# michael-fonder/M4Depth

Hardware: AMD Instinct MI355X
Metric: frames/s (higher is better)
Workload: dtype f32

## Files before the change

include/m4depth_hip.h:

```cpp
#ifndef M4DEPTH_HIP_H_
#define M4DEPTH_HIP_H_

#include <stdint.h>

#ifdef __cplusplus
extern "C" {
#endif

#define M4D_ABI_VERSION 6

int m4d_abi_version(void);
long long m4d_launch_count(void);
const char* m4d_build_info(void);


int m4d_backproject_fwd(const float* input, const float* coords, const int dims[6],
                        float* out, void* stream);

int m4d_backproject_bwd(const float* grad, const float* input, const float* coords,
                        const int dims[6], float* input_grad, float* coords_grad, void* stream);


int m4d_dense_image_warp(const float* image, const float* flow, int B, int H, int W, int C,
                         float* out, int32_t* index_out, void* stream);
// ... 181 lines not shown
                   float* parallax, float* depth, float* other, float* depth_state, void* stream);

int m4d_bias_act(const float* x, const float* bias, long long rows, int C, float slope,
                 float* out, void* stream);

int m4d_bias_act_padded(const float* x, const float* bias, int b, int h, int w, int C, float slope,
                        float* out, int out_h, int out_w, int off_y, int off_x, void* stream);

int m4d_conv3x3_bias_act(const float* x, const float* wp, const float* bias, int b, int h, int w,
                         int Cin, int Cout, int CoutPad, float slope, float* out, void* stream);
long long m4d_conv3x3_workspace_floats(int b, int h, int w, int CoutPad);
int m4d_conv3x3s_bias_act_ws(const float* x, const float* wp, const float* bias, int b, int h, int w,
                             int Cin, int Cout, int CoutPad, int stride, float slope, float* out,
                             float* workspace, long long workspace_floats, void* stream);
int m4d_conv3x3_bias_act_ws(const float* x, const float* wp, const float* bias, int b, int h, int w,
                            int Cin, int Cout, int CoutPad, float slope, float* out, float* workspace,
                            long long workspace_floats, void* stream);
int m4d_conv3x3_lat(const float* x, int s_in, long long x_slab_floats, const float* x_bias, float x_slope,
                    const void* wp, const float* bias, int b, int h, int w, int Cin, int Cout, float slope,
                    int mt, int kw, int s_out, float* out, long long out_slab_floats, void* stream);
int m4d_conv3x3s_lat(const float* x, int s_in, long long x_slab_floats, const float* x_bias, float x_slope,
                     const void* wp, const float* bias, int b, int h, int w, int Cin, int Cout, int stride, float slope,
                     int mt, int kw, int s_out, float* out, long long out_slab_floats, void* stream);
int m4d_partial_finish(const float* x, int s_in, long long x_slab_floats, const float* bias, float slope,
                       long long pixels, int C, float* out, void* stream);

int m4d_conv3x3_small_bias_act(const float* x, const float* wp, const float* bias, int b, int h, int w,
                               int Cin, int Cout, int CoutPad, float slope, float* out, void* stream);
int m4d_conv3x3s_small_bias_act(const float* x, const float* wp, const float* bias, int b, int h, int w,
                                int Cin, int Cout, int CoutPad, int stride, float slope, float* out, void* stream);
int m4d_conv3x3_small6_bias_act(const float* x, const void* wp6, const float* bias, int b, int h, int w,
                                int Cin, int Cout, int CoutPad, float slope, float* out, void* stream);

long long m4d_dinl_workspace_floats(int b, int C);
int m4d_dinl_fwd_padded(const float* x, const float* scale, const float* bias, int b, int h, int w, int C,
                        float slope, float* workspace, float* out, int out_h, int out_w, int off_y,
                        int off_x, void* stream);
int m4d_dinl_fwd(const float* x, const float* scale, const float* bias, int b, int h, int w, int C,
                 float slope, float* workspace, float* out, void* stream);

int m4d_enc_level0_fwd(const float* images, int bsz, long long stride_b, long long stride_t,
                       const float* w1_hwio, const float* bias1, const float* dn_scale, const float* dn_bias,
                       float dn_slope, const float* w2_hwio, const float* bias2, float slope,
                       int b, int h, int w, float* workspace, float* out, void* stream);
int m4d_enc_level0_stats(const float* images, int bsz, long long stride_b, long long stride_t,
                         const float* w1_hwio, const float* bias1, int b, int h, int w, float* workspace,
// ... 36 lines not shown
```

m4depth_amd/_lib.py:

```python
from __future__ import annotations

import ctypes
import os

import torch

_HERE = os.path.dirname(os.path.abspath(__file__))
LIB_FLAVOUR = os.environ.get("M4D_LIB_FLAVOUR", "product")
LIB_PATH = os.path.join(_HERE, "libm4depth_hip_exp.so" if LIB_FLAVOUR == "experiments" else "libm4depth_hip.so")

ABI_VERSION = 6

_c_fp = ctypes.c_void_p
_c_int = ctypes.c_int
_c_f = ctypes.c_float

class NormLevel(ctypes.Structure):
    _fields_ = [("x", ctypes.c_void_p), ("out", ctypes.c_void_p), ("pixels", ctypes.c_longlong), ("C", ctypes.c_int),
                ("nbre_cuts", ctypes.c_int)]


class ResetLevel(ctypes.Structure):
    _fields_ = [("features", ctypes.c_void_p), ("state_features", ctypes.c_void_p), ("depth_state", ctypes.c_void_p),
                ("parallax", ctypes.c_void_p), ("depth", ctypes.c_void_p), ("other", ctypes.c_void_p),
# ... 35 lines not shown
    "m4d_decode_rgb8_resize": [_c_fp, _c_int, _c_int, _c_int, _c_int, _c_int, _c_fp, _c_fp],
    "m4d_decode_depth_resize": [_c_fp, _c_int, _c_int, _c_int, _c_int, _c_int, _c_int, _c_fp, ctypes.POINTER(_c_int),
                                _c_fp, _c_fp],
    "m4d_normalize_cuts": [_c_fp, _c_int, _c_int, _c_int, _c_int, _c_int, _c_fp, _c_fp],
    "m4d_resize_bilinear_v1": [_c_fp, _c_int, _c_int, _c_int, _c_int, _c_int, _c_int, _c_f, _c_fp, _c_fp],
    "m4d_resize_nearest": [_c_fp, _c_int, _c_int, _c_int, _c_int, _c_int, _c_int, _c_fp, _c_fp],
    "m4d_bias_act": [_c_fp, _c_fp, ctypes.c_longlong, _c_int, _c_f, _c_fp, _c_fp],
    "m4d_dinl_fwd": [_c_fp, _c_fp, _c_fp, _c_int, _c_int, _c_int, _c_int, _c_f, _c_fp, _c_fp, _c_fp],
    "m4d_dinl_fwd_padded": [_c_fp, _c_fp, _c_fp, _c_int, _c_int, _c_int, _c_int, _c_f, _c_fp, _c_fp,
                            _c_int, _c_int, _c_int, _c_int, _c_fp],
    "m4d_bias_act_padded": [_c_fp, _c_fp, _c_int, _c_int, _c_int, _c_int, _c_f, _c_fp, _c_int, _c_int, _c_int, _c_int, _c_fp],
    "m4d_conv3x3_bias_act": [_c_fp, _c_fp, _c_fp, _c_int, _c_int, _c_int, _c_int, _c_int, _c_int, _c_f, _c_fp, _c_fp],
    "m4d_conv3x3_bias_act_ws": [_c_fp, _c_fp, _c_fp, _c_int, _c_int, _c_int, _c_int, _c_int, _c_int, _c_f, _c_fp,
                                _c_fp, ctypes.c_longlong, _c_fp],
    "m4d_conv3x3s_bias_act_ws": [_c_fp, _c_fp, _c_fp, _c_int, _c_int, _c_int, _c_int, _c_int, _c_int, _c_int, _c_f,
                                 _c_fp, _c_fp, ctypes.c_longlong, _c_fp],
    "m4d_conv3x3_small_bias_act": [_c_fp, _c_fp, _c_fp, _c_int, _c_int, _c_int, _c_int, _c_int, _c_int, _c_f, _c_fp, _c_fp],
    "m4d_conv3x3s_small_bias_act": [_c_fp, _c_fp, _c_fp, _c_int, _c_int, _c_int, _c_int, _c_int, _c_int, _c_int, _c_f, _c_fp, _c_fp],
    "m4d_conv3x3_small6_bias_act": [_c_fp, _c_fp, _c_fp, _c_int, _c_int, _c_int, _c_int, _c_int, _c_int, _c_f, _c_fp, _c_fp],
    "m4d_conv3x3_lat": [_c_fp, _c_int, ctypes.c_longlong, _c_fp, _c_f, _c_fp, _c_fp, _c_int, _c_int, _c_int, _c_int, _c_int, _c_f,
                        _c_int, _c_int, _c_int, _c_fp, ctypes.c_longlong, _c_fp],
    "m4d_conv3x3s_lat": [_c_fp, _c_int, ctypes.c_longlong, _c_fp, _c_f, _c_fp, _c_fp, _c_int, _c_int, _c_int, _c_int, _c_int, _c_int,
                         _c_f, _c_int, _c_int, _c_int, _c_fp, ctypes.c_longlong, _c_fp],
    "m4d_partial_finish": [_c_fp, _c_int, ctypes.c_longlong, _c_fp, _c_f, ctypes.c_longlong, _c_int, _c_fp, _c_fp],
    "m4d_conv3x3_wino_bias_act": [_c_fp, _c_fp, _c_fp, _c_int, _c_int, _c_int, _c_int, _c_int, _c_int, _c_f, _c_fp, _c_fp],
    "m4d_conv3x3_wino2_bias_act": [_c_fp, _c_fp, _c_fp, _c_int, _c_int, _c_int, _c_int, _c_int, _c_int, _c_f, _c_fp, _c_fp],
    "m4d_conv3x3_wino6_bias_act": [_c_fp, _c_fp, _c_fp, _c_int, _c_int, _c_int, _c_int, _c_int, _c_int, _c_f, _c_fp, _c_fp],
    "m4d_conv3x3_wino6_bias_act_k": [_c_fp, _c_fp, _c_fp, _c_int, _c_int, _c_int, _c_int, _c_int, _c_int, _c_f, _c_fp, _c_int, _c_fp],
    "m4d_conv3x3_wino6_bias_act_ks": [_c_fp, _c_fp, _c_fp, _c_int, _c_int, _c_int, _c_int, _c_int, _c_int, _c_f, _c_fp, _c_int,
                                      _c_int, _c_int, _c_fp],
    "m4d_conv3x3_winof16_bias_act_ks": [_c_fp, _c_fp, _c_fp, _c_int, _c_int, _c_int, _c_int, _c_int, _c_int, _c_f, _c_fp,
                                        _c_int, _c_int, _c_fp],
    "m4d_enc_head_fwd": [_c_fp, _c_int, ctypes.c_longlong, ctypes.c_longlong, _c_fp, _c_fp, _c_int, _c_int, _c_int, _c_int,
                         _c_fp, _c_fp, _c_fp],
    "m4d_enc_level0_stats": [_c_fp, _c_int, ctypes.c_longlong, ctypes.c_longlong, _c_fp, _c_fp, _c_int, _c_int, _c_int, _c_fp, _c_fp, _c_fp,
                             _c_fp],
    "m4d_enc_level0_apply": [_c_fp, _c_int, ctypes.c_longlong, ctypes.c_longlong, _c_fp, _c_fp, _c_fp, _c_fp, _c_fp, _c_fp, _c_f, _c_fp,
                             _c_fp, _c_f, _c_int, _c_int, _c_int, _c_fp, _c_fp],
    "m4d_enc_level0_fwd": [_c_fp, _c_int, ctypes.c_longlong, ctypes.c_longlong, _c_fp, _c_fp, _c_fp, _c_fp, _c_f, _c_fp, _c_fp, _c_f,
                           _c_int, _c_int, _c_int, _c_fp, _c_fp, _c_fp],
    "m4d_conv3x3s2_dinl_bias_act": [_c_fp, _c_fp, _c_fp, _c_fp, _c_fp, _c_f, _c_fp, _c_fp, _c_int, _c_int, _c_int, _c_int, _c_int,
                                    _c_f, _c_fp, _c_fp],
    "m4d_refiner_tail": [_c_fp, _c_fp, _c_fp, _c_fp, _c_fp, _c_fp, _c_int, _c_fp, _c_fp, _c_fp, _c_int, _c_int, _c_int, _c_f,
                         _c_fp, _c_fp, _c_fp, _c_fp, _c_fp],
    "m4d_refiner_tail6": [_c_fp, _c_fp, _c_fp, _c_fp, _c_fp, _c_fp, _c_int, _c_fp, _c_fp, _c_fp, _c_int, _c_int, _c_int, _c_f,
                          _c_fp, _c_fp, _c_fp, _c_fp, _c_fp],
# ... 153 lines not shown
```

m4depth_amd/csrc/m4d_convlat.hip:

```cpp
#include <cstdlib>
#include "m4d_common.h"
#include "../../include/m4depth_hip.h"

namespace {

typedef float lat_f32x16 __attribute__((ext_vector_type(16)));
typedef __bf16 lat_bf16x8 __attribute__((ext_vector_type(8)));

struct LatArgs {
  const float* x; long long x_slab; int s_in;
  const float* x_bias; float x_slope;
  const unsigned char* wp;
  const float* bias; float slope;
  float* out; long long out_slab; int s_out;
  int b, h, w, Cin, Cout, n_chunks, n_groups, tiles_x, tiles_y;
  int cgw_log2, chunks_per_slice;
  int oh, ow, pad_y, pad_x;
};

constexpr int kLatRow = 24;

template <int SIN, int HW, int HP>
__device__ __forceinline__ void lat_stage(const LatArgs& a, float* lds_a, int t, int bi, int gy0, int gx0, int c0, int n_st) {
  constexpr int IB = SIN >= 3 ? 2 : 4;
  const int n_items = n_st * HP * 4;
  for (int base = 0; base < n_items; base += 256 * IB) {
    float4 v[IB][SIN];
    int dst[IB], ch[IB];
    bool ok[IB];
#pragma unroll
    for (int i = 0; i < IB; ++i) {
      const int idx = base + i * 256 + t;
      const int idc = min(idx, n_items - 1);
      const int j = idc / (HP * 4), rem = idc - j * (HP * 4);
      const int hp = rem >> 2, q = rem & 3;
      const int gy = gy0 + hp / HW, gx = gx0 + hp % HW;
      ch[i] = (c0 + j) * 16 + 4 * q;
      ok[i] = idx < n_items && gy >= 0 && gy < a.h && gx >= 0 && gx < a.w && ch[i] < a.Cin;
      dst[i] = idx < n_items ? (j * HP + hp) * kLatRow + 2 * q : -1;
      const long long off = (((long long)bi * a.h + min(max(gy, 0), a.h - 1)) * a.w + min(max(gx, 0), a.w - 1)) * a.Cin
                            + min(ch[i], a.Cin - 4);
#pragma unroll
      for (int s = 0; s < SIN; ++s) v[i][s] = *reinterpret_cast<const float4*>(a.x + s * a.x_slab + off);
// ... 165 lines not shown
    v.x += bb.x; v.y += bb.y; v.z += bb.z; v.w += bb.w;
    v.x = v.x > 0.f ? v.x : v.x * slope; v.y = v.y > 0.f ? v.y : v.y * slope;
    v.z = v.z > 0.f ? v.z : v.z * slope; v.w = v.w > 0.f ? v.w : v.w * slope;
    reinterpret_cast<float4*>(out)[i] = v;
  }
}

template <int MTX, int MTY, int STRIDE, bool MW = false>
int lat_launch(const LatArgs& a, int kw_in, hipStream_t s) {
  constexpr int HP = ((8 * MTX - 1) * STRIDE + 3) * ((4 * MTY - 1) * STRIDE + 3), MT = MTX * MTY;
  const int kw = MW ? 1 : kw_in;
  const int cgw = MW ? 1 : 4 / kw;
  const size_t lds_a = (size_t)2 * kw * HP * kLatRow * 4;
  const size_t lds_r = (size_t)(kw - 1) * cgw * MT * 16 * 64 * 4;
  const size_t lds = lds_a > lds_r ? lds_a : lds_r;
  if (lds > 64 * 1024) M4D_LDS_OPT_IN(&conv3x3_lat_kernel<MTX, MTY, STRIDE, MW>);
  const dim3 grid((unsigned)(a.b * a.tiles_x * a.tiles_y), (unsigned)((a.n_groups + cgw - 1) / cgw), (unsigned)a.s_out);
  m4d_launch(conv3x3_lat_kernel<MTX, MTY, STRIDE, MW>, grid, dim3(256), lds, s, a);
  return 0;
}

}

static int lat_make_args(LatArgs& a, int& kw, const float* x, int s_in, long long x_slab_floats, const float* x_bias, float x_slope,
                         const void* wp, const float* bias, int b, int h, int w, int Cin, int Cout, int stride, float slope,
                         int mt, int s_out, float* out, long long out_slab_floats) {
  M4D_CHECK_ARG(x && wp && bias && out && b > 0 && h > 0 && w > 0 && (stride == 1 || stride == 2));
  M4D_CHECK_ARG(Cin >= 16 && Cin % 4 == 0 && Cout >= 1);
  const int oh = (h + stride - 1) / stride, ow = (w + stride - 1) / stride;
  M4D_CHECK_ARG(s_in >= 1 && s_in <= 4 && (s_in == 1 || x_slab_floats >= (long long)b * h * w * Cin));
  M4D_CHECK_ARG(s_out >= 1 && (s_out == 1 || out_slab_floats >= (long long)b * oh * ow * Cout));
  M4D_CHECK_ARG((mt == 1 || mt == 2 || mt == 4 || mt == 8) && (kw == 1 || kw == 2 || kw == 4));
  if (mt == 8) kw = 1;
  a.x = x; a.x_slab = x_slab_floats; a.s_in = s_in; a.x_bias = x_bias; a.x_slope = x_slope;
  a.wp = reinterpret_cast<const unsigned char*>(wp); a.bias = bias; a.slope = slope;
  a.out = out; a.out_slab = out_slab_floats; a.s_out = s_out;
  a.b = b; a.h = h; a.w = w; a.Cin = Cin; a.Cout = Cout; a.oh = oh; a.ow = ow;
  a.pad_y = ((oh - 1) * stride + 3 - h > 0 ? (oh - 1) * stride + 3 - h : 0) / 2;
  a.pad_x = ((ow - 1) * stride + 3 - w > 0 ? (ow - 1) * stride + 3 - w : 0) / 2;
  a.n_chunks = (Cin + 15) / 16; a.n_groups = (Cout + 31) / 32;
  M4D_CHECK_ARG(s_out <= a.n_chunks);
  a.cgw_log2 = kw == 1 ? 2 : (kw == 2 ? 1 : 0);
  a.chunks_per_slice = (a.n_chunks + s_out - 1) / s_out;
  M4D_CHECK_ARG((long long)(s_out - 1) * a.chunks_per_slice < a.n_chunks);
  const int mtx = mt >= 4 ? 2 : 1, mty = mt >= 2 ? 2 : 1;
  a.tiles_x = (ow + 8 * mtx - 1) / (8 * mtx); a.tiles_y = (oh + 4 * mty - 1) / (4 * mty);
  const size_t lds_a = (size_t)2 * kw * ((8 * mtx - 1) * stride + 3) * ((4 * mty - 1) * stride + 3) * kLatRow * 4;
  M4D_CHECK_ARG(lds_a <= 160 * 1024);
  return 0;
}

static int lat_launch_any(const float* x, int s_in, long long x_slab_floats, const float* x_bias, float x_slope,
                          const void* wp, const float* bias, int b, int h, int w, int Cin, int Cout, int stride, float slope,
                          int mt, int kw, int s_out, float* out, long long out_slab_floats, void* stream) {
  LatArgs a;
  const int rc = lat_make_args(a, kw, x, s_in, x_slab_floats, x_bias, x_slope, wp, bias, b, h, w, Cin, Cout, stride, slope, mt, s_out,
                               out, out_slab_floats);
  if (rc) return rc;
  hipStream_t s = (hipStream_t)stream;
  int rl;
  if (stride == 1) {
    if (mt == 1) rl = lat_launch<1, 1, 1>(a, kw, s);
    else if (mt == 2) rl = lat_launch<1, 2, 1>(a, kw, s);
    else if (mt == 4) rl = lat_launch<2, 2, 1>(a, kw, s);
    else rl = lat_launch<2, 2, 1, true>(a, kw, s);
  } else {
    if (mt == 1) rl = lat_launch<1, 1, 2>(a, kw, s);
    else if (mt == 2) rl = lat_launch<1, 2, 2>(a, kw, s);
    else if (mt == 4) rl = lat_launch<2, 2, 2>(a, kw, s);
    else rl = lat_launch<2, 2, 2, true>(a, kw, s);
  }
  if (rl) return rl;
  return M4D_LAUNCH_RESULT();
}
// ... 26 lines not shown
```

m4depth_amd/network.py:

```python
from __future__ import annotations

import ctypes
from collections import namedtuple

import numpy as np
import torch

from . import network_ops as nops
from ._lib import lib, dptr, stream_ptr, check, as_f32
from .synthetic import ENCODER_CHANNELS, REFINER_CHANNELS, f_input_channels, nbre_cuts_for

M4depthAblationParameters = namedtuple('M4depthAblationParameters',
                                       ('DINL', 'SNCV', 'time_recurr', 'normalize_features',
                                        'subdivide_features', 'level_memory'),
                                       defaults=(True, True, True, True, True, True))

_CV_ACCUM = {"fp32_round": 0, "fp16_seq": 1}

import os as _os

kernel_timer = None
debug_tap = None
winograd_conv = _os.environ.get("M4D_WINOGRAD", "1") == "1"

# ... 45 lines not shown
    n32 = -(-cout // 32)
    t16 = b * (-(-h // 16)) * (-(-w // 16))
    if conv_arith in _SPLIT_ARITHS and cin % 16 == 0 and cin >= 32 and cout >= wino6_min_cout and t16 * (-(-cout // 64)) >= wino6_min_workgroups:
        return 6
    if cin % 4 == 0 and t16 * n32 >= winograd2_min_workgroups:
        return 2
    t8 = b * (-(-h // 8)) * (-(-w // 16))
    if cout % 64 == 0 and t8 * (cout // 64) >= 400:
        return 1
    if cout >= 96 and 400 <= t8 * n32 <= 3000:
        return 1
    return 0


pad_refiner_input = _os.environ.get("M4D_PAD_REFINER_INPUT", "1") == "1"

small_map_conv_pixels = int(_os.environ.get("M4D_CONV_SMALL_PX", "2048"))
small_map_stride2 = _os.environ.get("M4D_CONV_SMALL_S2", "1") == "1"

lat_conv_max_pixels = int(_os.environ.get("M4D_LAT_CONV_PX", "2048"))
lat_conv_narrow_max_pixels = int(_os.environ.get("M4D_LAT_CONV_NARROW_PX", "0"))
lat_conv_s2_max_pixels = int(_os.environ.get("M4D_LAT_CONV_S2_PX", "0"))
lat_conv_mw_max_pixels = int(_os.environ.get("M4D_LAT_CONV_MW_PX", "0"))

fused_cost_volumes = _os.environ.get("M4D_FUSED_COST_VOLUMES", "1") == "1"
small_level_front = _os.environ.get("M4D_SMALL_LEVEL_FRONT", "1") == "1"
fused_level_front = _os.environ.get("M4D_FUSED_LEVEL_FRONT", "1") == "1"

fused_front = _os.environ.get("M4D_FUSED_FRONT", "1") == "1"
fused_front_min_pixels = int(_os.environ.get("M4D_FUSED_FRONT_MIN_PX", "0"))
fused_front_coarse_min_pixels = int(_os.environ.get("M4D_FUSED_FRONT_COARSE_MIN_PX", "6000"))

fused_encoder_head = _os.environ.get("M4D_FUSED_ENCODER_HEAD", "1") == "1"

fused_refiner_tail = _os.environ.get("M4D_FUSED_TAIL", "1") == "1"

level_pipeline_streams = int(_os.environ.get("M4D_LEVEL_PIPELINE", "8"))
_pf = _os.environ.get("M4D_PIPE_FORK_FRAMES", "1,2")
pipeline_fork_frames = None if _pf == "all" else {int(v) for v in _pf.split(",") if v.strip() != ""}
pipeline_skip_implied_encoder_wait = _os.environ.get("M4D_PIPE_SKIP_ENC_WAIT", "1") == "1"
pipeline_merge_reset_frame = _os.environ.get("M4D_PIPE_MERGE_RESET", "1") == "1"
wino6_stagger_us = int(_os.environ.get("M4D_WINO6_STAGGER_US", "9"))
wino6_stagger_phases = int(_os.environ.get("M4D_WINO6_STAGGER_PHASES", "16"))
wino6_stagger_min_wg = int(_os.environ.get("M4D_WINO6_STAGGER_MIN_WG", "200"))
wino6_stagger_max_batch = int(_os.environ.get("M4D_WINO6_STAGGER_MAX_BATCH", "4"))
wino6_stagger_autotune = _os.environ.get("M4D_STAGGER_AUTOTUNE", "1") == "1"
# ... 133 lines not shown
        def build():
            wu, cpad = nops.pack_conv_weights_winograd(self._hwio_numpy(cin_pad), chunk=chunk)
            return torch.from_numpy(wu).to(self.weight.device), cpad
        return self._cache.get(("wino", chunk, cin_pad), _stamp(self.weight), build)

    def _packed_weights_small6(self, cin_pad=None):
        if cin_pad is not None and cin_pad == self.weight.shape[1]:
            cin_pad = None

        def build():
            wp, cpad = nops.pack_conv_weights_small6(self._hwio_numpy(cin_pad))
            return torch.from_numpy(wp.view("int16")).to(self.weight.device), cpad
        return self._cache.get(("small6", cin_pad), _stamp(self.weight), build)

    def _packed_weights_lat(self, cin_pad=None):
        if cin_pad is not None and cin_pad == self.weight.shape[1]:
            cin_pad = None

        def build():
            wp = nops.pack_conv_weights_lat(self._hwio_numpy(cin_pad))
            return torch.from_numpy(wp.view("int16")).to(self.weight.device)
        return self._cache.get(("lat", cin_pad), _stamp(self.weight), build)

    def lat_eligible(self, b, h, w, cin):
        if not (self.small_maps_ok and conv_arith in _SPLIT_ARITHS and cin >= 16 and cin % 4 == 0 and self.stride in (1, 2)):
            return False
        eff_b = self.dispatch_batch if self.per_image_dispatch else b
        if self.stride == 2:
            opx = eff_b * (-(-h // 2)) * (-(-w // 2))
            return self._lat_mw(b, h, w, cin) or (small_map_stride2 and opx <= lat_conv_s2_max_pixels)
        limit = max(lat_conv_max_pixels, lat_conv_narrow_max_pixels) if self.out_channels <= 32 else lat_conv_max_pixels
        return eff_b * h * w <= limit

    def _lat_mw(self, b, h, w, cin):
        eff_b = self.dispatch_batch if self.per_image_dispatch else b
        return (self.stride == 2 and cin % 16 == 0 and cin <= 64 and self.out_channels <= 64
                and small_map_conv_pixels < eff_b * (-(-h // 2)) * (-(-w // 2)) <= lat_conv_mw_max_pixels)

    def _packed_weights_wino6(self, cin_pad=None):
        if cin_pad is not None and cin_pad == self.weight.shape[1]:
            cin_pad = None

        def build():
            wu, cpad = nops.pack_conv_weights_wino6(self._hwio_numpy(cin_pad))
            return torch.from_numpy(wu.view("int16")).to(self.weight.device), cpad
        return self._cache.get(("wino6", cin_pad), _stamp(self.weight), build)
# ... 17 lines not shown
        return (ph // 2, ph - ph // 2), (pw // 2, pw - pw // 2)

    def launch_stagger_us(self, b, h, w):
        us = wino6_stagger_us if self.wino6_stagger_us is None else self.wino6_stagger_us
        if us <= 0 or b > wino6_stagger_max_batch:
            return 0
        units = b * (-(-h // 16)) * (-(-w // 16)) * (-(-self.out_channels // 64))
        return int(us) if units >= wino6_stagger_min_wg else 0

    def forward(self, x_nhwc, slope=None, final=True):
        if isinstance(x_nhwc, nops.PartialAct) and not self.lat_eligible(*x_nhwc.shape):
            x_nhwc = x_nhwc.dense()
        if not x_nhwc.is_cuda:
            raise RuntimeError("m4depth_amd convolutions run on the GPU only (libm4depth_hip.so): got a CPU tensor; "
                               "there is no CPU fallback")
        if self.weight is None:
            self._build(x_nhwc.shape[-1], x_nhwc.device)
        if self.stride not in (1, 2):
            raise ValueError(f"stride {self.stride} is not supported by the HIP convolution")
        b_, h_, w_, cin_ = x_nhwc.shape
        act = 1.0 if slope is None else slope
        eff_b = self.dispatch_batch if self.per_image_dispatch else b_
        if self.lat_eligible(b_, h_, w_, cin_):
            wl = self._packed_weights_lat(cin_)
            cfg = nops.lat_config(eff_b, h_, w_, cin_, self.out_channels, final, self.stride, mw=self._lat_mw(b_, h_, w_, cin_))
            return _timed("conv", self.tag, lambda: nops.conv3x3_lat(x_nhwc, wl, self.bias, self.out_channels, act, config=cfg,
                                                                     stride=self.stride))
        wino = _use_winograd(eff_b, h_, w_, cin_, self.out_channels, self.stride)
        if wino == 6:
            f16 = conv_arith == "f16x2"
            wu, cpad = self._packed_weights_winof16(cin_) if f16 else self._packed_weights_wino6(cin_)
            stag = self.launch_stagger_us(b_, h_, w_)
            kern = wino6_kernel
            if not f16 and kern == 0 and wino6_pair_min_units > 0 and b_ <= wino6_stagger_max_batch and cin_ >= 32:
                units = b_ * (-(-h_ // 16)) * (-(-w_ // 16)) * (cpad // 64)
                if wino6_pair_min_units <= units < int(lib.m4d_wino6_persistent_min_units()):
                    kern = 16 + max(1, min(wino6_pair_units, 15))
            return _timed("conv", self.tag, lambda: nops.conv3x3_wino6_bias_act(
                x_nhwc, wu, self.bias, self.out_channels, cpad, act, kernel=kern, stagger_us=stag,
                stagger_phases=wino6_stagger_phases, arith=conv_arith))
        if wino:
            wu, cpad = self._packed_weights_winograd(16 if wino == 1 else 8, cin_)
            fn = nops.conv3x3_wino_bias_act if wino == 1 else nops.conv3x3_wino2_bias_act
            return _timed("conv", self.tag, lambda: fn(x_nhwc, wu, self.bias, self.out_channels, cpad, act))
        wp, cpad = self._packed_weights(cin_)
        if (self.small_maps_ok and self.stride == 1 and eff_b * h_ * w_ <= small_map_conv_pixels and 16 <= cin_ <= 256
                and cin_ % 4 == 0):
            if small_conv_split:
# ... 658 lines not shown
            with torch.no_grad():
                dn.scale.copy_(sc)
                dn.bias.copy_(bi)
        else:
            dn.scale = torch.nn.Parameter(sc, requires_grad=False)
            dn.bias = torch.nn.Parameter(bi, requires_grad=False)
        for lvl in self.d_estimator.levels:
            convs = list(lvl.disp_refiner.prep_conv_layers) + list(lvl.disp_refiner.est_d_conv_layers)
            for i, conv in enumerate(convs):
                conv.load_hwio(weights[f"lvl.{lvl.lvl_depth}.conv.{i}.kernel"], weights[f"lvl.{lvl.lvl_depth}.conv.{i}.bias"], device)
        return self.prepack()

    def prepack(self):
        for conv in self.modules():
            if isinstance(conv, _Conv3x3SameTF) and conv.weight is not None and conv.weight.is_cuda:
                cin = conv.weight.shape[1]
                conv._packed_weights()
                if small_conv_split and conv.small_maps_ok and conv.stride == 1 and 16 <= cin <= 256 and cin % 4 == 0:
                    conv._packed_weights_small6()
                if conv.small_maps_ok and conv_arith in _SPLIT_ARITHS and cin >= 16 and cin % 4 == 0 and (
                        (conv.stride == 1 and max(lat_conv_max_pixels, lat_conv_narrow_max_pixels) > 0)
                        or (conv.stride == 2 and max(lat_conv_s2_max_pixels, lat_conv_mw_max_pixels) > 0)):
                    conv._packed_weights_lat()
                if cin == 3 or (conv.stride == 2 and cin == 16 and conv.out_channels == 16):
                    conv._hwio_device()
                if conv.stride == 1 and cin >= 16 and cin % 2 == 0:
                    conv._packed_weights_winograd(16)
                    if cin % 4 == 0:
                        conv._packed_weights_winograd(8)
                    if cin % 16 == 0 and cin >= 32 and conv.out_channels >= min(wino6_min_cout, 32):
                        conv._packed_weights_wino6()
                        conv._packed_weights_winof16()
        for lvl in self.d_estimator.levels:
            convs = list(lvl.disp_refiner.prep_conv_layers) + list(lvl.disp_refiner.est_d_conv_layers)
            c0 = convs[0] if convs else None
            if pad_refiner_input and c0 is not None and c0.weight is not None and c0.weight.is_cuda and c0.weight.shape[1] % 8 != 0:
                cin_pad = (c0.weight.shape[1] + 7) // 8 * 8
                c0._packed_weights(cin_pad)
                c0._packed_weights_winograd(16, cin_pad)
                c0._packed_weights_winograd(8, cin_pad)
                if small_conv_split and cin_pad <= 256:
                    c0._packed_weights_small6(cin_pad)
                if conv_arith in _SPLIT_ARITHS and lat_conv_max_pixels > 0:
                    c0._packed_weights_lat(cin_pad)
                if cin_pad % 16 == 0 and cin_pad >= 32 and c0.out_channels >= min(wino6_min_cout, 32):
                    c0._packed_weights_wino6(cin_pad)
                    c0._packed_weights_winof16(cin_pad)
            if len(convs) == 7 and convs[5].weight is not None and convs[5].weight.is_cuda \
                    and tuple(convs[5].weight.shape[:2]) == (16, 32) and tuple(convs[6].weight.shape[:2]) == (5, 16):
                lvl._tail_weights(convs, tail_split and conv_arith in _SPLIT_ARITHS)
        return self

    def invalidate_packed(self):
        for conv in self.modules():
            if isinstance(conv, _Conv3x3SameTF):
                conv.invalidate_packed()
        return self.prepack()

    def weights_stamp(self):
        return tuple((c.weight.data_ptr(), c.weight._version) for c in self.modules()
                     if isinstance(c, _Conv3x3SameTF) and c.weight is not None)

    def load_tf_checkpoint(self, prefix_or_dir, device):
        from . import tf_checkpoint as TC
        prefix = prefix_or_dir
        if _os.path.isdir(prefix_or_dir):
            prefix = TC.latest_checkpoint(prefix_or_dir)
# ... 733 lines not shown
```

m4depth_amd/network_ops.py:

```python
from __future__ import annotations

import ctypes

import torch

from ._lib import lib, dptr, stream_ptr, check, as_f32


def normalize_cuts(x, nbre_cuts, out=None):
    x = as_f32(x, "x")
    b, h, w, C = x.shape
    if C % nbre_cuts != 0:
        raise ValueError(f"nbre_cuts={nbre_cuts} does not divide the {C} feature channels")
    if out is None:
        out = torch.empty_like(x)
    check(lib.m4d_normalize_cuts(dptr(x, "x"), b, h, w, C, int(nbre_cuts), dptr(out, "out"), stream_ptr()),
          "m4d_normalize_cuts")
    return out


def resize_bilinear_v1(x, out_h, out_w, mul=1.0):
    x = as_f32(x, "x")
    b, ih, iw, c = x.shape
    out = torch.empty((b, out_h, out_w, c), dtype=torch.float32, device=x.device)
# ... 345 lines not shown
    k = np.asarray(kernel_hwio, dtype=np.float32)
    assert k.shape[:2] == (3, 3)
    cin, cout = k.shape[2], k.shape[3]
    nch = -(-cin // 16)
    cpad = -(-cout // 32) * 32
    full = np.zeros((9, nch * 16, cpad), np.float32)
    full[:, :cin, :cout] = k.reshape(9, cin, cout)
    parts = split_bf16x3(full).reshape(3, 9, nch, 16, cpad)
    return np.ascontiguousarray(parts.transpose(2, 1, 4, 0, 3)), cpad


def pack_conv_weights_lat(kernel_hwio):
    import numpy as np
    k = np.asarray(kernel_hwio, dtype=np.float32)
    assert k.shape[:2] == (3, 3)
    cin, cout = k.shape[2], k.shape[3]
    nch, ng = -(-cin // 16), -(-cout // 32)
    full = np.zeros((9, nch * 16, ng * 32), np.float32)
    full[:, :cin, :cout] = k.reshape(9, cin, cout)
    parts = split_bf16x3(full).reshape(3, 9, nch, 2, 8, ng, 32)
    return np.ascontiguousarray(parts.transpose(5, 2, 1, 0, 3, 6, 4)).reshape(ng, nch, 9, 3, 64, 8)


class PartialAct:

    def __init__(self, slabs, bias, slope):
        self.slabs, self.bias, self.slope = slabs, bias, 1.0 if slope is None else float(slope)

    @property
    def shape(self):
        return self.slabs.shape[1:]

    @property
    def is_cuda(self):
        return self.slabs.is_cuda

    @property
    def device(self):
        return self.slabs.device

    def dense(self):
        S, b, h, w, C = self.slabs.shape
        out = torch.empty((b, h, w, C), dtype=torch.float32, device=self.slabs.device)
        check(lib.m4d_partial_finish(dptr(self.slabs, "slabs"), S, b * h * w * C, dptr(self.bias, "bias"), self.slope,
                                     b * h * w, C, dptr(out), stream_ptr()), "m4d_partial_finish")
        return out
# ... 31 lines not shown
        kw //= 2
    while wgs(mt, kw) > lat_max_workgroups and mt < 4 and fits(mt * 2, kw):
        mt *= 2
    return mt, kw, s_out


def conv3x3_lat(x, wp, bias, cout, slope=0.1, final=False, config=None, stride=1):
    if isinstance(x, PartialAct):
        xs, s_in, x_bias, x_slope = x.slabs, x.slabs.shape[0], x.bias, x.slope
        b, h, w, cin = x.shape
        slab = b * h * w * cin
    else:
        xs = as_f32(x, "x")
        s_in, x_bias, x_slope = 1, None, 1.0
        b, h, w, cin = xs.shape
        slab = 0
    mt, kw, s_out = config if config is not None else lat_config(b, h, w, cin, cout, final, stride)
    act = 1.0 if slope is None else float(slope)
    oh, ow = -(-h // stride), -(-w // stride)
    out = torch.empty((s_out, b, oh, ow, cout), dtype=torch.float32, device=xs.device)
    check(lib.m4d_conv3x3s_lat(dptr(xs, "x"), s_in, slab, dptr(x_bias, "x_bias"), float(x_slope), dptr(wp, "wp", torch.int16),
                               dptr(bias, "bias"), b, h, w, cin, int(cout), int(stride), act, mt, kw, s_out, dptr(out),
                               b * oh * ow * int(cout), stream_ptr()), "m4d_conv3x3s_lat")
    return out[0] if s_out == 1 else PartialAct(out, bias, act)


def conv3x3_small6_bias_act(x, wp6, bias, cout, cout_pad, slope=0.1):
    x = as_f32(x, "x")
    b, h, w, cin = x.shape
    out = torch.empty((b, h, w, cout), dtype=torch.float32, device=x.device)
    check(lib.m4d_conv3x3_small6_bias_act(dptr(x, "x"), dptr(wp6, "wp6", torch.int16), dptr(bias, "bias"), b, h, w, cin, int(cout),
                                          int(cout_pad), float(slope), dptr(out), stream_ptr()), "m4d_conv3x3_small6_bias_act")
    return out


def conv3x3_winof16_bias_act(x, wuh, bias, cout, cout_pad, slope=0.1, stagger_us=0, stagger_phases=16):
    x = as_f32(x, "x")
    b, h, w, cin = x.shape
    out = torch.empty((b, h, w, cout), dtype=torch.float32, device=x.device)
    check(lib.m4d_conv3x3_winof16_bias_act_ks(dptr(x, "x"), dptr(wuh, "wuh", torch.int16), dptr(bias, "bias"), b, h, w, cin,
                                              int(cout), int(cout_pad), float(slope), dptr(out), int(stagger_us),
                                              int(stagger_phases), stream_ptr()),
          "m4d_conv3x3_winof16_bias_act_ks")
    return out


# ... 224 lines not shown
```

Before: 1752.

## Add f16x2 split-precision variant of latency conv3x3 with per-pixel exponent scaling

```diff
diff --git a/include/m4depth_hip.h b/include/m4depth_hip.h
--- a/include/m4depth_hip.h
+++ b/include/m4depth_hip.h
@@ -227,6 +227,9 @@
 int m4d_conv3x3s_lat(const float* x, int s_in, long long x_slab_floats, const float* x_bias, float x_slope,
                      const void* wp, const float* bias, int b, int h, int w, int Cin, int Cout, int stride, float slope,
                      int mt, int kw, int s_out, float* out, long long out_slab_floats, void* stream);
+int m4d_conv3x3_lat_f16(const float* x, int s_in, long long x_slab_floats, const float* x_bias, float x_slope,
+                        const void* wp, const float* bias, int b, int h, int w, int Cin, int Cout, float slope,
+                        int mt, int kw, int s_out, float* out, long long out_slab_floats, void* stream);
 int m4d_partial_finish(const float* x, int s_in, long long x_slab_floats, const float* bias, float slope,
                        long long pixels, int C, float* out, void* stream);
 
diff --git a/m4depth_amd/_lib.py b/m4depth_amd/_lib.py
--- a/m4depth_amd/_lib.py
+++ b/m4depth_amd/_lib.py
@@ -81,6 +81,8 @@
                         _c_int, _c_int, _c_int, _c_fp, ctypes.c_longlong, _c_fp],
     "m4d_conv3x3s_lat": [_c_fp, _c_int, ctypes.c_longlong, _c_fp, _c_f, _c_fp, _c_fp, _c_int, _c_int, _c_int, _c_int, _c_int, _c_int,
                          _c_f, _c_int, _c_int, _c_int, _c_fp, ctypes.c_longlong, _c_fp],
+    "m4d_conv3x3_lat_f16": [_c_fp, _c_int, ctypes.c_longlong, _c_fp, _c_f, _c_fp, _c_fp, _c_int, _c_int, _c_int, _c_int, _c_int,
+                            _c_f, _c_int, _c_int, _c_int, _c_fp, ctypes.c_longlong, _c_fp],
     "m4d_partial_finish": [_c_fp, _c_int, ctypes.c_longlong, _c_fp, _c_f, ctypes.c_longlong, _c_int, _c_fp, _c_fp],
     "m4d_conv3x3_wino_bias_act": [_c_fp, _c_fp, _c_fp, _c_int, _c_int, _c_int, _c_int, _c_int, _c_int, _c_f, _c_fp, _c_fp],
     "m4d_conv3x3_wino2_bias_act": [_c_fp, _c_fp, _c_fp, _c_int, _c_int, _c_int, _c_int, _c_int, _c_int, _c_f, _c_fp, _c_fp],
diff --git a/m4depth_amd/csrc/m4d_convlat.h b/m4depth_amd/csrc/m4d_convlat.h
--- /dev/null
+++ b/m4depth_amd/csrc/m4d_convlat.h
@@ -0,0 +1,50 @@
+#pragma once
+#include "m4d_common.h"
+
+namespace {
+
+typedef float lat_f32x16 __attribute__((ext_vector_type(16)));
+typedef __bf16 lat_bf16x8 __attribute__((ext_vector_type(8)));
+
+struct LatArgs {
+  const float* x; long long x_slab; int s_in;
+  const float* x_bias; float x_slope;
+  const unsigned char* wp;
+  const float* bias; float slope;
+  float* out; long long out_slab; int s_out;
+  int b, h, w, Cin, Cout, n_chunks, n_groups, tiles_x, tiles_y;
+  int cgw_log2, chunks_per_slice;
+  int oh, ow, pad_y, pad_x;
+};
+
+constexpr int kLatRow = 24;
+
+}
+
+static int lat_make_args(LatArgs& a, int& kw, const float* x, int s_in, long long x_slab_floats, const float* x_bias, float x_slope,
+                         const void* wp, const float* bias, int b, int h, int w, int Cin, int Cout, int stride, float slope,
+                         int mt, int s_out, float* out, long long out_slab_floats) {
+  M4D_CHECK_ARG(x && wp && bias && out && b > 0 && h > 0 && w > 0 && (stride == 1 || stride == 2));
+  M4D_CHECK_ARG(Cin >= 16 && Cin % 4 == 0 && Cout >= 1);
+  const int oh = (h + stride - 1) / stride, ow = (w + stride - 1) / stride;
+  M4D_CHECK_ARG(s_in >= 1 && s_in <= 4 && (s_in == 1 || x_slab_floats >= (long long)b * h * w * Cin));
+  M4D_CHECK_ARG(s_out >= 1 && (s_out == 1 || out_slab_floats >= (long long)b * oh * ow * Cout));
+  M4D_CHECK_ARG((mt == 1 || mt == 2 || mt == 4 || mt == 8) && (kw == 1 || kw == 2 || kw == 4));
+  if (mt == 8) kw = 1;
+  a.x = x; a.x_slab = x_slab_floats; a.s_in = s_in; a.x_bias = x_bias; a.x_slope = x_slope;
+  a.wp = reinterpret_cast<const unsigned char*>(wp); a.bias = bias; a.slope = slope;
+  a.out = out; a.out_slab = out_slab_floats; a.s_out = s_out;
+  a.b = b; a.h = h; a.w = w; a.Cin = Cin; a.Cout = Cout; a.oh = oh; a.ow = ow;
+  a.pad_y = ((oh - 1) * stride + 3 - h > 0 ? (oh - 1) * stride + 3 - h : 0) / 2;
+  a.pad_x = ((ow - 1) * stride + 3 - w > 0 ? (ow - 1) * stride + 3 - w : 0) / 2;
+  a.n_chunks = (Cin + 15) / 16; a.n_groups = (Cout + 31) / 32;
+  M4D_CHECK_ARG(s_out <= a.n_chunks);
+  a.cgw_log2 = kw == 1 ? 2 : (kw == 2 ? 1 : 0);
+  a.chunks_per_slice = (a.n_chunks + s_out - 1) / s_out;
+  M4D_CHECK_ARG((long long)(s_out - 1) * a.chunks_per_slice < a.n_chunks);
+  const int mtx = mt >= 4 ? 2 : 1, mty = mt >= 2 ? 2 : 1;
+  a.tiles_x = (ow + 8 * mtx - 1) / (8 * mtx); a.tiles_y = (oh + 4 * mty - 1) / (4 * mty);
+  const size_t lds_a = (size_t)2 * kw * ((8 * mtx - 1) * stride + 3) * ((4 * mty - 1) * stride + 3) * kLatRow * 4;
+  M4D_CHECK_ARG(lds_a <= 160 * 1024);
+  return 0;
+}
diff --git a/m4depth_amd/csrc/m4d_convlat.hip b/m4depth_amd/csrc/m4d_convlat.hip
--- a/m4depth_amd/csrc/m4d_convlat.hip
+++ b/m4depth_amd/csrc/m4d_convlat.hip
@@ -1,24 +1,9 @@
 #include <cstdlib>
 #include "m4d_common.h"
+#include "m4d_convlat.h"
 #include "../../include/m4depth_hip.h"
 
 namespace {
-
-typedef float lat_f32x16 __attribute__((ext_vector_type(16)));
-typedef __bf16 lat_bf16x8 __attribute__((ext_vector_type(8)));
-
-struct LatArgs {
-  const float* x; long long x_slab; int s_in;
-  const float* x_bias; float x_slope;
-  const unsigned char* wp;
-  const float* bias; float slope;
-  float* out; long long out_slab; int s_out;
-  int b, h, w, Cin, Cout, n_chunks, n_groups, tiles_x, tiles_y;
-  int cgw_log2, chunks_per_slice;
-  int oh, ow, pad_y, pad_x;
-};
-
-constexpr int kLatRow = 24;
 
 template <int SIN, int HW, int HP>
 __device__ __forceinline__ void lat_stage(const LatArgs& a, float* lds_a, int t, int bi, int gy0, int gx0, int c0, int n_st) {
@@ -230,34 +215,6 @@
 
 }
 
-static int lat_make_args(LatArgs& a, int& kw, const float* x, int s_in, long long x_slab_floats, const float* x_bias, float x_slope,
-                         const void* wp, const float* bias, int b, int h, int w, int Cin, int Cout, int stride, float slope,
-                         int mt, int s_out, float* out, long long out_slab_floats) {
-  M4D_CHECK_ARG(x && wp && bias && out && b > 0 && h > 0 && w > 0 && (stride == 1 || stride == 2));
-  M4D_CHECK_ARG(Cin >= 16 && Cin % 4 == 0 && Cout >= 1);
-  const int oh = (h + stride - 1) / stride, ow = (w + stride - 1) / stride;
-  M4D_CHECK_ARG(s_in >= 1 && s_in <= 4 && (s_in == 1 || x_slab_floats >= (long long)b * h * w * Cin));
-  M4D_CHECK_ARG(s_out >= 1 && (s_out == 1 || out_slab_floats >= (long long)b * oh * ow * Cout));
-  M4D_CHECK_ARG((mt == 1 || mt == 2 || mt == 4 || mt == 8) && (kw == 1 || kw == 2 || kw == 4));
-  if (mt == 8) kw = 1;
-  a.x = x; a.x_slab = x_slab_floats; a.s_in = s_in; a.x_bias = x_bias; a.x_slope = x_slope;
-  a.wp = reinterpret_cast<const unsigned char*>(wp); a.bias = bias; a.slope = slope;
-  a.out = out; a.out_slab = out_slab_floats; a.s_out = s_out;
-  a.b = b; a.h = h; a.w = w; a.Cin = Cin; a.Cout = Cout; a.oh = oh; a.ow = ow;
-  a.pad_y = ((oh - 1) * stride + 3 - h > 0 ? (oh - 1) * stride + 3 - h : 0) / 2;
-  a.pad_x = ((ow - 1) * stride + 3 - w > 0 ? (ow - 1) * stride + 3 - w : 0) / 2;
-  a.n_chunks = (Cin + 15) / 16; a.n_groups = (Cout + 31) / 32;
-  M4D_CHECK_ARG(s_out <= a.n_chunks);
-  a.cgw_log2 = kw == 1 ? 2 : (kw == 2 ? 1 : 0);
-  a.chunks_per_slice = (a.n_chunks + s_out - 1) / s_out;
-  M4D_CHECK_ARG((long long)(s_out - 1) * a.chunks_per_slice < a.n_chunks);
-  const int mtx = mt >= 4 ? 2 : 1, mty = mt >= 2 ? 2 : 1;
-  a.tiles_x = (ow + 8 * mtx - 1) / (8 * mtx); a.tiles_y = (oh + 4 * mty - 1) / (4 * mty);
-  const size_t lds_a = (size_t)2 * kw * ((8 * mtx - 1) * stride + 3) * ((4 * mty - 1) * stride + 3) * kLatRow * 4;
-  M4D_CHECK_ARG(lds_a <= 160 * 1024);
-  return 0;
-}
-
 static int lat_launch_any(const float* x, int s_in, long long x_slab_floats, const float* x_bias, float x_slope,
                           const void* wp, const float* bias, int b, int h, int w, int Cin, int Cout, int stride, float slope,
                           int mt, int kw, int s_out, float* out, long long out_slab_floats, void* stream) {
diff --git a/m4depth_amd/csrc/m4d_convlat_f16.hip b/m4depth_amd/csrc/m4d_convlat_f16.hip
--- /dev/null
+++ b/m4depth_amd/csrc/m4d_convlat_f16.hip
@@ -0,0 +1,265 @@
+#include <cstdlib>
+#include "m4d_common.h"
+#include "m4d_convlat.h"
+#include "../../include/m4depth_hip.h"
+
+namespace {
+
+typedef _Float16 lat_f16x8 __attribute__((ext_vector_type(8)));
+typedef unsigned lat_u32x4 __attribute__((ext_vector_type(4)));
+
+constexpr int kRowF = 20;
+constexpr int kFragF16 = 18 * 1024;
+
+__device__ __forceinline__ void lat_split2_pair(float v0, float v1, float S, unsigned& hi, unsigned& lo) {
+  asm("v_fma_mixlo_f16 %0, %1, %2, 0" : "=v"(hi) : "v"(v0), "v"(S));
+  asm("v_fma_mixhi_f16 %0, %1, %2, 0" : "+v"(hi) : "v"(v1), "v"(S));
+  asm("v_fma_mixlo_f16 %0, %1, %2, -%3 op_sel_hi:[0,0,1]" : "=v"(lo) : "v"(v0), "v"(S), "v"(hi));
+  asm("v_fma_mixhi_f16 %0, %1, %2, -%3 op_sel:[0,0,1] op_sel_hi:[0,0,1]" : "+v"(lo) : "v"(v1), "v"(S), "v"(hi));
+}
+
+__device__ __forceinline__ unsigned lat_abs_bits(float v) { return min(__float_as_uint(v) & 0x7fffffffu, 0x7f7fffffu); }
+
+template <int SIN, int HW, int HP>
+__device__ __forceinline__ void lat_stage_f16(const LatArgs& a, float* halo, unsigned* pm, int t, int bi, int gy0, int gx0, int c0,
+                                              int n_st) {
+  constexpr int IB = SIN >= 3 ? 2 : 4;
+  const int n_items = n_st * HP * 4;
+  for (int base = 0; base < n_items; base += 256 * IB) {
+    float4 v[IB][SIN];
+    int item[IB], ch[IB];
+    bool ok[IB];
+#pragma unroll
+    for (int i = 0; i < IB; ++i) {
+      const int idx = base + i * 256 + t;
+      const int idc = min(idx, n_items - 1);
+      const int j = idc / (HP * 4), rem = idc - j * (HP * 4);
+      const int hp = rem >> 2, q = rem & 3;
+      const int gy = gy0 + hp / HW, gx = gx0 + hp % HW;
+      ch[i] = (c0 + j) * 16 + 4 * q;
+      ok[i] = idx < n_items && gy >= 0 && gy < a.h && gx >= 0 && gx < a.w && ch[i] < a.Cin;
+      item[i] = idx < n_items ? idx >> 2 : -1;
+      const long long off = (((long long)bi * a.h + min(max(gy, 0), a.h - 1)) * a.w + min(max(gx, 0), a.w - 1)) * a.Cin
+                            + min(ch[i], a.Cin - 4);
+#pragma unroll
+      for (int s = 0; s < SIN; ++s) v[i][s] = *reinterpret_cast<const float4*>(a.x + s * a.x_slab + off);
+    }
+#pragma unroll
+    for (int i = 0; i < IB; ++i) {
+      float e[4] = {v[i][0].x, v[i][0].y, v[i][0].z, v[i][0].w};
+#pragma unroll
+      for (int s = 1; s < SIN; ++s) { e[0] += v[i][s].x; e[1] += v[i][s].y; e[2] += v[i][s].z; e[3] += v[i][s].w; }
+      if (a.x_bias != nullptr) {
+        const float4 bb = *reinterpret_cast<const float4*>(a.x_bias + min(ch[i], a.Cin - 4));
+        const float bv[4] = {bb.x, bb.y, bb.z, bb.w};
+#pragma unroll
+        for (int k = 0; k < 4; ++k) { const float u = e[k] + bv[k]; e[k] = u > 0.f ? u : u * a.x_slope; }
+      }
+#pragma unroll
+      for (int k = 0; k < 4; ++k) e[k] = ok[i] ? e[k] : 0.f;
+      unsigned u = max(max(lat_abs_bits(e[0]), lat_abs_bits(e[1])), max(lat_abs_bits(e[2]), lat_abs_bits(e[3])));
+      u = max(u, (unsigned)__builtin_amdgcn_update_dpp(0, (int)u, 0xb1, 0xf, 0xf, false));
+      u = max(u, (unsigned)__builtin_amdgcn_update_dpp(0, (int)u, 0x4e, 0xf, 0xf, false));
+      if (item[i] >= 0) {
+        *reinterpret_cast<float4*>(halo + item[i] * kRowF + 4 * (t & 3)) = make_float4(e[0], e[1], e[2], e[3]);
+        if ((t & 3) == 0) pm[item[i]] = u;
+      }
+    }
+  }
+}
+
+template <int MTX, int MTY>
+__global__ void __launch_bounds__(256, 1)
+conv3x3_lat_f16_kernel(const LatArgs a) {
+  extern __shared__ __align__(16) float lds_dyn[];
+  constexpr int MT = MTX * MTY;
+  constexpr int TW = 8 * MTX, TH = 4 * MTY, HW = TW + 2, HP = HW * (TH + 2);
+  constexpr int kChunkF = HP * kRowF;
+  const int t = threadIdx.x, lane = t & 63;
+  const int wave = __builtin_amdgcn_readfirstlane(t >> 6);
+  const int cgw = 1 << a.cgw_log2, kw = 4 >> a.cgw_log2;
+  const int cg = wave & (cgw - 1), ks = wave >> a.cgw_log2;
+  const int bx = blockIdx.x, by = blockIdx.y, bz = blockIdx.z;
+  const int tiles = a.tiles_x * a.tiles_y;
+  const int bi = bx / tiles, tile = bx - bi * tiles;
+  const int ty0 = (tile / a.tiles_x) * TH, tx0 = (tile % a.tiles_x) * TW;
+  const int g = by * cgw + cg;
+  const bool active = g < a.n_groups;
+  const int c_begin = bz * a.chunks_per_slice;
+  const int c_end = min(a.n_chunks, c_begin + a.chunks_per_slice);
+  const int n_slice = max(c_end - c_begin, 0);
+  const int rounds = (n_slice + kw - 1) / kw;
+  const int n = lane & 31, kh = lane >> 5;
+  const int co = g * 32 + n;
+  float* halo = lds_dyn;
+  unsigned* pm = reinterpret_cast<unsigned*>(lds_dyn + 2 * kw * kChunkF);
+  int* ts = reinterpret_cast<int*>(pm + 2 * kw * HP) + wave * MT * 32;
+  const float my_bias = (a.s_out == 1 && active && co < a.Cout) ? a.bias[co] : 0.f;
+  const int gc = min(g, a.n_groups - 1);
+  const int my_t = reinterpret_cast<const short*>(a.wp + (long long)a.n_groups * a.n_chunks * kFragF16)[gc * 32 + n];
+
+  lat_f32x16 acc[MT];
+#pragma unroll
+  for (int m = 0; m < MT; ++m)
+#pragma unroll
+    for (int r = 0; r < 16; ++r) acc[m][r] = 0.f;
+
+  const unsigned char* wg = a.wp + ((long long)gc * a.n_chunks) * kFragF16 + lane * 16;
+
+  for (int r0 = 0; r0 < rounds; r0 += 2) {
+    float4 bq[2][2][9];
+    bool valid[2];
+#pragma unroll
+    for (int q = 0; q < 2; ++q) {
+      const int c = c_begin + (r0 + q) * kw + ks;
+      valid[q] = active && (r0 + q) < rounds && c < c_end;
+      const unsigned char* wc = wg + (long long)min(c, a.n_chunks - 1) * kFragF16;
+      if (valid[q]) {
+#pragma unroll
+        for (int p = 0; p < 2; ++p)
+#pragma unroll
+          for (int tp = 0; tp < 9; ++tp) bq[q][p][tp] = *reinterpret_cast<const float4*>(wc + (tp * 2 + p) * 1024);
+      }
+    }
+    const int c0 = c_begin + r0 * kw;
+    const int n_st = min(2 * kw, c_end - c0);
+    switch (a.s_in) {
+      case 1: lat_stage_f16<1, HW, HP>(a, halo, pm, t, bi, ty0 - 1, tx0 - 1, c0, n_st); break;
+      case 2: lat_stage_f16<2, HW, HP>(a, halo, pm, t, bi, ty0 - 1, tx0 - 1, c0, n_st); break;
+      case 3: lat_stage_f16<3, HW, HP>(a, halo, pm, t, bi, ty0 - 1, tx0 - 1, c0, n_st); break;
+      default: lat_stage_f16<4, HW, HP>(a, halo, pm, t, bi, ty0 - 1, tx0 - 1, c0, n_st); break;
+    }
+    __syncthreads();
+    if (valid[0]) {
+      float Sc[MT];
+#pragma unroll
+      for (int m = 0; m < MT; ++m) {
+        const int my = m / MTX, mx = m % MTX;
+        const int hp0 = (my * 4 + (n >> 3)) * HW + mx * 8 + (n & 7);
+        unsigned um = 0;
+#pragma unroll
+        for (int q = 0; q < 2; ++q) {
+          if (valid[q]) {
+            const unsigned* pq = pm + (q * kw + ks) * HP + hp0;
+#pragma unroll
+            for (int tp = 0; tp < 9; ++tp) um = max(um, pq[(tp / 3) * HW + tp % 3]);
+          }
+        }
+        const int s = min(139 - (int)(um >> 23), 126);
+        Sc[m] = __uint_as_float((unsigned)(s + 127) << 23);
+        if (kh == 0) ts[m * 32 + n] = -s;
+      }
+      lat_f32x16 part[MT];
+#pragma unroll
+      for (int m = 0; m < MT; ++m)
+#pragma unroll
+        for (int r = 0; r < 16; ++r) part[m][r] = 0.f;
+#pragma unroll
+      for (int q = 0; q < 2; ++q) {
+        if (valid[q]) {
+          const float* ac = halo + (q * kw + ks) * kChunkF + kh * 8;
+#pragma unroll
+          for (int tp = 0; tp < 9; ++tp) {
+            const lat_f16x8 bh = __builtin_bit_cast(lat_f16x8, bq[q][0][tp]);
+            const lat_f16x8 bl = __builtin_bit_cast(lat_f16x8, bq[q][1][tp]);
+#pragma unroll
+            for (int m = 0; m < MT; ++m) {
+              const int my = m / MTX, mx = m % MTX;
+              const float* ap = ac + ((my * 4 + (n >> 3) + tp / 3) * HW + mx * 8 + (n & 7) + tp % 3) * kRowF;
+              const float4 x0 = *reinterpret_cast<const float4*>(ap);
+              const float4 x1 = *reinterpret_cast<const float4*>(ap + 4);
+              unsigned ah[4], al[4];
+              lat_split2_pair(x0.x, x0.y, Sc[m], ah[0], al[0]);
+              lat_split2_pair(x0.z, x0.w, Sc[m], ah[1], al[1]);
+              lat_split2_pair(x1.x, x1.y, Sc[m], ah[2], al[2]);
+              lat_split2_pair(x1.z, x1.w, Sc[m], ah[3], al[3]);
+              const lat_f16x8 h = __builtin_bit_cast(lat_f16x8, lat_u32x4{ah[0], ah[1], ah[2], ah[3]});
+              const lat_f16x8 l = __builtin_bit_cast(lat_f16x8, lat_u32x4{al[0], al[1], al[2], al[3]});
+              part[m] = __builtin_amdgcn_mfma_f32_32x32x16_f16(h, bl, part[m], 0, 0, 0);
+              part[m] = __builtin_amdgcn_mfma_f32_32x32x16_f16(l, bh, part[m], 0, 0, 0);
+              part[m] = __builtin_amdgcn_mfma_f32_32x32x16_f16(h, bh, part[m], 0, 0, 0);
+            }
+          }
+        }
+      }
+#pragma unroll
+      for (int m = 0; m < MT; ++m)
+#pragma unroll
+        for (int g4 = 0; g4 < 4; ++g4) {
+          const int4 ne = *reinterpret_cast<const int4*>(ts + m * 32 + 8 * g4 + 4 * kh);
+          acc[m][4 * g4 + 0] += __builtin_ldexpf(part[m][4 * g4 + 0], ne.x - my_t);
+          acc[m][4 * g4 + 1] += __builtin_ldexpf(part[m][4 * g4 + 1], ne.y - my_t);
+          acc[m][4 * g4 + 2] += __builtin_ldexpf(part[m][4 * g4 + 2], ne.z - my_t);
+          acc[m][4 * g4 + 3] += __builtin_ldexpf(part[m][4 * g4 + 3], ne.w - my_t);
+        }
+    }
+    if (r0 + 2 < rounds) __syncthreads();
+  }
+  if (kw > 1) {
+    __syncthreads();
+    float* red = lds_dyn;
+    if (ks > 0) {
+#pragma unroll
+      for (int m = 0; m < MT; ++m)
+#pragma unroll
+        for (int r = 0; r < 16; ++r) red[((((ks - 1) * cgw + cg) * MT + m) * 16 + r) * 64 + lane] = acc[m][r];
+    }
+    __syncthreads();
+    if (ks == 0) {
+      for (int k = 1; k < kw; ++k)
+#pragma unroll
+        for (int m = 0; m < MT; ++m)
+#pragma unroll
+          for (int r = 0; r < 16; ++r) acc[m][r] += red[((((k - 1) * cgw + cg) * MT + m) * 16 + r) * 64 + lane];
+    }
+  }
+  if (ks == 0 && active && co < a.Cout) {
+    float* op = a.out + bz * a.out_slab + (long long)bi * a.oh * a.ow * a.Cout + co;
+    const bool final_out = a.s_out == 1;
+#pragma unroll
+    for (int m = 0; m < MT; ++m) {
+      const int my = m / MTX, mx = m % MTX;
+#pragma unroll
+      for (int r = 0; r < 16; ++r) {
+        const int mr = (r & 3) + 8 * (r >> 2) + 4 * kh;
+        const int oy = ty0 + my * 4 + (mr >> 3), ox = tx0 + mx * 8 + (mr & 7);
+        if (oy < a.oh && ox < a.ow) {
+          float v = acc[m][r];
+          if (final_out) { v += my_bias; v = v > 0.f ? v : v * a.slope; }
+          op[((long long)oy * a.ow + ox) * a.Cout] = v;
+        }
+      }
+    }
+  }
+}
+
+template <int MTX, int MTY>
+int lat_f16_launch(const LatArgs& a, int kw, hipStream_t s) {
+  constexpr int HP = (8 * MTX + 2) * (4 * MTY + 2), MT = MTX * MTY;
+  const int cgw = 4 / kw;
+  const size_t lds_a = (size_t)2 * kw * HP * (kRowF + 1) * 4 + 4 * MT * 32 * 4;
+  const size_t lds_r = (size_t)(kw - 1) * cgw * MT * 16 * 64 * 4;
+  const size_t lds = lds_a > lds_r ? lds_a : lds_r;
+  M4D_CHECK_ARG(lds <= 160 * 1024);
+  if (lds > 64 * 1024) M4D_LDS_OPT_IN(&conv3x3_lat_f16_kernel<MTX, MTY>);
+  const dim3 grid((unsigned)(a.b * a.tiles_x * a.tiles_y), (unsigned)((a.n_groups + cgw - 1) / cgw), (unsigned)a.s_out);
+  m4d_launch(conv3x3_lat_f16_kernel<MTX, MTY>, grid, dim3(256), lds, s, a);
+  return 0;
+}
+
+}
+
+extern "C" int m4d_conv3x3_lat_f16(const float* x, int s_in, long long x_slab_floats, const float* x_bias, float x_slope,
+                                   const void* wp, const float* bias, int b, int h, int w, int Cin, int Cout, float slope,
+                                   int mt, int kw, int s_out, float* out, long long out_slab_floats, void* stream) {
+  M4D_CHECK_ARG(mt == 1 || mt == 2 || mt == 4);
+  M4D_CHECK_ARG((((uintptr_t)wp) & 15u) == 0);
+  LatArgs a;
+  const int rc = lat_make_args(a, kw, x, s_in, x_slab_floats, x_bias, x_slope, wp, bias, b, h, w, Cin, Cout, 1, slope, mt, s_out,
+                               out, out_slab_floats);
+  if (rc) return rc;
+  hipStream_t s = (hipStream_t)stream;
+  const int rl = mt == 1 ? lat_f16_launch<1, 1>(a, kw, s) : mt == 2 ? lat_f16_launch<1, 2>(a, kw, s) : lat_f16_launch<2, 2>(a, kw, s);
+  if (rl) return rl;
+  return M4D_LAUNCH_RESULT();
+}
diff --git a/m4depth_amd/network.py b/m4depth_amd/network.py
--- a/m4depth_amd/network.py
+++ b/m4depth_amd/network.py
@@ -91,6 +91,9 @@
 lat_conv_narrow_max_pixels = int(_os.environ.get("M4D_LAT_CONV_NARROW_PX", "0"))
 lat_conv_s2_max_pixels = int(_os.environ.get("M4D_LAT_CONV_S2_PX", "0"))
 lat_conv_mw_max_pixels = int(_os.environ.get("M4D_LAT_CONV_MW_PX", "0"))
+lat_arith = _os.environ.get("M4D_LAT_ARITH", "f16x2")
+if lat_arith not in _SPLIT_ARITHS:
+    raise ValueError(f"M4D_LAT_ARITH must be 'f16x2' or 'bf16x3', not {lat_arith!r}")
 
 fused_cost_volumes = _os.environ.get("M4D_FUSED_COST_VOLUMES", "1") == "1"
 small_level_front = _os.environ.get("M4D_SMALL_LEVEL_FRONT", "1") == "1"
@@ -270,6 +273,18 @@
             return torch.from_numpy(wp.view("int16")).to(self.weight.device)
         return self._cache.get(("lat", cin_pad), _stamp(self.weight), build)
 
+    def _packed_weights_lat_f16(self, cin_pad=None):
+        if cin_pad is not None and cin_pad == self.weight.shape[1]:
+            cin_pad = None
+
+        def build():
+            wp = nops.pack_conv_weights_lat_f16(self._hwio_numpy(cin_pad))
+            return torch.from_numpy(wp.view("int16")).to(self.weight.device)
+        return self._cache.get(("lat_f16", cin_pad), _stamp(self.weight), build)
+
+    def lat_f16(self, mw=False):
+        return conv_arith == "f16x2" and lat_arith == "f16x2" and self.stride == 1 and not mw
+
     def lat_eligible(self, b, h, w, cin):
         if not (self.small_maps_ok and conv_arith in _SPLIT_ARITHS and cin >= 16 and cin % 4 == 0 and self.stride in (1, 2)):
             return False
@@ -333,8 +348,13 @@
         act = 1.0 if slope is None else slope
         eff_b = self.dispatch_batch if self.per_image_dispatch else b_
         if self.lat_eligible(b_, h_, w_, cin_):
+            mw = self._lat_mw(b_, h_, w_, cin_)
+            cfg = nops.lat_config(eff_b, h_, w_, cin_, self.out_channels, final, self.stride, mw=mw)
+            if self.lat_f16(mw):
+                wl = self._packed_weights_lat_f16(cin_)
+                return _timed("conv", self.tag, lambda: nops.conv3x3_lat_f16(x_nhwc, wl, self.bias, self.out_channels, act,
+                                                                         config=cfg))
             wl = self._packed_weights_lat(cin_)
-            cfg = nops.lat_config(eff_b, h_, w_, cin_, self.out_channels, final, self.stride, mw=self._lat_mw(b_, h_, w_, cin_))
             return _timed("conv", self.tag, lambda: nops.conv3x3_lat(x_nhwc, wl, self.bias, self.out_channels, act, config=cfg,
                                                                      stride=self.stride))
         wino = _use_winograd(eff_b, h_, w_, cin_, self.out_channels, self.stride)
@@ -1039,6 +1059,8 @@
                         (conv.stride == 1 and max(lat_conv_max_pixels, lat_conv_narrow_max_pixels) > 0)
                         or (conv.stride == 2 and max(lat_conv_s2_max_pixels, lat_conv_mw_max_pixels) > 0)):
                     conv._packed_weights_lat()
+                    if conv.stride == 1:
+                        conv._packed_weights_lat_f16()
                 if cin == 3 or (conv.stride == 2 and cin == 16 and conv.out_channels == 16):
                     conv._hwio_device()
                 if conv.stride == 1 and cin >= 16 and cin % 2 == 0:
@@ -1060,6 +1082,7 @@
                     c0._packed_weights_small6(cin_pad)
                 if conv_arith in _SPLIT_ARITHS and lat_conv_max_pixels > 0:
                     c0._packed_weights_lat(cin_pad)
+                    c0._packed_weights_lat_f16(cin_pad)
                 if cin_pad % 16 == 0 and cin_pad >= 32 and c0.out_channels >= min(wino6_min_cout, 32):
                     c0._packed_weights_wino6(cin_pad)
                     c0._packed_weights_winof16(cin_pad)
diff --git a/m4depth_amd/network_ops.py b/m4depth_amd/network_ops.py
--- a/m4depth_amd/network_ops.py
+++ b/m4depth_amd/network_ops.py
@@ -391,6 +391,26 @@
     return np.ascontiguousarray(parts.transpose(5, 2, 1, 0, 3, 6, 4)).reshape(ng, nch, 9, 3, 64, 8)
 
 
+def pack_conv_weights_lat_f16(kernel_hwio):
+    import numpy as np
+    k = np.asarray(kernel_hwio, dtype=np.float32)
+    assert k.shape[:2] == (3, 3)
+    cin, cout = k.shape[2], k.shape[3]
+    nch, ng = -(-cin // 16), -(-cout // 32)
+    full = np.zeros((9, nch * 16, ng * 32), np.float32)
+    full[:, :cin, :cout] = k.reshape(9, cin, cout)
+    if not np.isfinite(full).all():
+        raise ValueError("pack_conv_weights_lat_f16: non-finite weight")
+    amax = np.abs(full).max(axis=(0, 1)).astype(np.float64)
+    texp = np.where(amax > 0, 15 - np.frexp(amax)[1], 0).astype(np.int64)
+    scaled = full.astype(np.float64) * np.ldexp(1.0, texp)[None, None, :]
+    hi = scaled.astype(np.float16)
+    lo = (scaled - hi.astype(np.float64)).astype(np.float16)
+    parts = np.stack([hi, lo]).view(np.uint16).reshape(2, 9, nch, 2, 8, ng, 32)
+    w = np.ascontiguousarray(parts.transpose(5, 2, 1, 0, 3, 6, 4))
+    return np.concatenate([w.reshape(-1), texp.astype(np.int16).view(np.uint16)])
+
+
 class PartialAct:
 
     def __init__(self, slabs, bias, slope):
@@ -468,6 +488,25 @@
     check(lib.m4d_conv3x3s_lat(dptr(xs, "x"), s_in, slab, dptr(x_bias, "x_bias"), float(x_slope), dptr(wp, "wp", torch.int16),
                                dptr(bias, "bias"), b, h, w, cin, int(cout), int(stride), act, mt, kw, s_out, dptr(out),
                                b * oh * ow * int(cout), stream_ptr()), "m4d_conv3x3s_lat")
+    return out[0] if s_out == 1 else PartialAct(out, bias, act)
+
+
+def conv3x3_lat_f16(x, wp, bias, cout, slope=0.1, final=False, config=None):
+    if isinstance(x, PartialAct):
+        xs, s_in, x_bias, x_slope = x.slabs, x.slabs.shape[0], x.bias, x.slope
+        b, h, w, cin = x.shape
+        slab = b * h * w * cin
+    else:
+        xs = as_f32(x, "x")
+        s_in, x_bias, x_slope = 1, None, 1.0
+        b, h, w, cin = xs.shape
+        slab = 0
+    mt, kw, s_out = config if config is not None else lat_config(b, h, w, cin, cout, final)
+    act = 1.0 if slope is None else float(slope)
+    out = torch.empty((s_out, b, h, w, cout), dtype=torch.float32, device=xs.device)
+    check(lib.m4d_conv3x3_lat_f16(dptr(xs, "x"), s_in, slab, dptr(x_bias, "x_bias"), float(x_slope), dptr(wp, "wp", torch.int16),
+                                  dptr(bias, "bias"), b, h, w, cin, int(cout), act, mt, kw, s_out, dptr(out),
+                                  b * h * w * int(cout), stream_ptr()), "m4d_conv3x3_lat_f16")
     return out[0] if s_out == 1 else PartialAct(out, bias, act)
 
 
```

Result: faster. 1780 (median of 6 runs) (+1.6%).
